# zongh5a/MDF-Net

Measured on AMD Instinct MI355X. Metric: views/sec at DTU 1600x1200x5-view x4-scale, higher is better.
Workload: dtype f32; 1 GPU; DTU eval 1600x1184 (1600x1200 cropped as load/dtueval.py:34), 5 views, 3 cost-volume stages + x2 refine = 4 output scales, hypotheses (48,24,8), batch 1 per rank, seeded random weights (pth/dtu_29.pth is not available offline); parallelism=views sharded over 1 rank(s), no collective

## Files before the change

include/mdfnet_hip.h:

```cpp
#ifndef MDFNET_HIP_H
#define MDFNET_HIP_H

#include <stdint.h>

#ifdef __cplusplus
extern "C" {
#endif

#define MDF_ABI_VERSION 1

#define MDF_OK 0
#define MDF_EARG (-1)
#define MDF_EUNSUPPORTED (-2)
#define MDF_EHIP (-3)

#define MDF_FEA_NCHW 0
#define MDF_FEA_NHWC 1
#define MDF_VOL_NCDHW 0
#define MDF_VOL_NDHWC 1

#define MDF_MAX_SRC_VIEWS 16
#define MDF_MAX_FUSE_VIEWS 1024

int mdf_abi_version(void);
const char* mdf_last_error(void);
const char* mdf_last_launch(void);
int mdf_release_stream(void* stream);

int mdf_homo_warp_fwd(const float* src_fea, int fea_layout, const float* proj, const float* hypos,
                      int hypos_per_pixel, float* out, int out_layout, int B, int C, int D, int h, int w,
                      void* stream);

int mdf_warp_corner_indices(const float* proj, const float* hypos, int hypos_per_pixel, int32_t* x0y0,
                            int B, int D, int h, int w, void* stream);

int mdf_warp_aggregate_vec_fwd(const float* ref_fea, const float* const* src_feas, int fea_layout,
                               const float* proj, const float* hypos, int hypos_per_pixel,
                               const float* w_params, float* cost, int cost_layout, int B, int C, int G,
                               int D, int h, int w, int n_src, void* stream);

int mdf_warp_aggregate_pairdiff_fwd(const float* ref_diff, const float* const* src_diffs, int fea_layout,
                                    const float* proj, const float* hypos, int hypos_per_pixel,
                                    const float* w_params, float* cost, int cost_layout, int B, int G, int D,
                                    int h, int w, int n_src, void* stream);

int mdf_warp_aggregate_var_fwd(const float* ref_fea, const float* const* src_feas, int fea_layout,
                               const float* proj, const float* hypos, int hypos_per_pixel, float* cost,
                               int cost_layout, int B, int C, int D, int h, int w, int n_src, void* stream);

int mdf_conv3d_fwd(const float* x, const float* wpack, const float* alpha, const float* beta, const float* res,
                   float* y, int B, int Di, int Hi, int Wi, int Cin, int Cout, int stride, int transposed,
                   int relu, void* stream);

int64_t mdf_conv3d_packed_size(int Cin, int Cout);
int mdf_conv3d_pack_weights(const float* w, float* wpack, int Cin, int Cout, int transposed, void* stream);

int mdf_conv2d_fwd(const float* x, const float* wpack, const float* alpha, const float* beta, const float* res,
                   float res_scale, const float* res_up, float* y, int B, int H, int W, int Cin, int Cout, int ksize, int stride, int relu,
                   int planar_in, int pixel_shuffle2, void* stream);
int64_t mdf_conv_packed_size(int Cin, int Cout, int ntaps);
int mdf_conv_pack_weights(const float* w, float* wpack, int Cin, int Cout, int ntaps, void* stream);

int mdf_prob_softmax_regress_fwd(const float* x, const float* w, const float* hypos, int hypos_per_pixel,
                                 float* prob, float* depth, int B, int D, int h, int wd, int Cin, void* stream);
int mdf_prob_from_partials_fwd(const float* partials, const float* hypos, int hypos_per_pixel, float* prob, float* depth,
                               int B, int D, int h, int wd, void* stream);
int mdf_prob_fused_fwd(const float* x, const float* wpack, const float* hypos, int hypos_per_pixel, float* prob, float* depth,
                       int B, int D, int h, int wd, int Cin, void* stream);

int mdf_refine_tail_fwd(const float* x, const float* w1pack, const float* w2, const float* lo, const float* span, float* y,
                        int B, int H, int W, void* stream);

int mdf_conv2d_pair_fwd(const float* x, const float* w1pack, const float* alpha1, const float* beta1, const float* w2pack,
                        const float* alpha2, const float* beta2, float* y, int N, int H, int W, void* stream);

int mdf_conv1x1_heads_fwd(const float* x, int n_heads, const float* const* wpacks, const float* const* biases,
                          const float* const* res_ups, float* const* ys, const int* couts, int B, int H, int W, int Cin,
                          void* stream);

int mdf_refine_head_fwd(const float* depth, const float* lo, const float* span, const float* weight, float* y, int B, int H, int W,
                        void* stream);

int mdf_conv2d_res_pair_fwd(const float* x, const float* wa_pack, const float* wb_pack, float scale, float* y, int N, int H,
                            int W, void* stream);

int mdf_depth_regress_fwd(const float* prob, const float* hypos, int hypos_per_pixel, float* depth, int B, int D,
                          int h, int w, void* stream);

int mdf_confidence_fwd(const float* prob, float* conf, int64_t* idx_out, int B, int D, int h, int w, void* stream);
int mdf_confidence_up2_fwd(const float* prob, float* conf2, int B, int D, int h, int w, void* stream);
int mdf_range_affine_fwd(const float* x, const float* lo, const float* span, int mode, float* y, int B, long long n, void* stream);

int mdf_hypos_fit_fwd(int mode, const float* prob, const float* depth, const float* hypos, int hypos_per_pixel,
                      const float* fit_row, float* s_out, int B, int D, int h, int w, void* stream);
int mdf_hypos_from_fit_fwd(int mode, const float* s, const float* depth, const float* range, float log_thresh,
                           float* hypos_out, int B, int D_out, int h, int w, int upsample, void* stream);

int mdf_consistency_fuse_fwd(const float* depth_ref, const float* conf, const float* const* src_depths, const float* mats,
                             int n_src, int h, int w, float photo_threshold, int nconditions, float thre1, float thre2,
                             float* depth_avg, unsigned char* masks, unsigned short* view_masks, float* rep_out, void* stream);

long long mdf_consensus_fuse_workspace(int n, int h, int w);
int mdf_consensus_fuse_fwd(const float* depths, const unsigned char* colors, const float* cams, int n, int h, int w, float f,
                           float disp_thresh, int num_consistent, void* workspace, float* xyz, unsigned char* rgb,
                           long long capacity, int* view_counts, long long* total, void* stream);
int mdf_consensus_compact(void* workspace, int n, int h, int w, float* xyz, unsigned char* rgb, long long capacity, void* stream);

#define MDF_PCD_MAX_SOURCES 64
#define MDF_PCD_STEP_VIS1 1
#define MDF_PCD_STEP_FUSION 2
#define MDF_PCD_STEP_VIS2 3
#define MDF_PCD_STEP_AVE 4
#define MDF_PCD_STEP_VIS3 5
#define MDF_PCD_STEP_SEG 6
long long mdf_pcd_fuse_workspace(int n, int h, int w, int v);
int mdf_pcd_fuse_fwd(float* depths, unsigned char* masks, const float* cams, const int* srcs, int n, int h, int w, int v, int need,
                     int first_step, int last_step, void* workspace, int* view_counts, long long* total, void* stream);
int mdf_pcd_compact(const float* depths, const unsigned char* masks, const unsigned char* rgb, const float* cams, int n, int h,
                    int w, int v, void* workspace, float* xyz, unsigned char* rgb_out, float* dirs, long long capacity,
                    void* stream);

long long mdf_pts_index_workspace(long long n);
int mdf_pts_index_build(const double* pts, long long n, void* index, long long index_bytes, void* stream);
int mdf_pts_nn_dist(const void* index, long long n, long long index_bytes, const void* qindex, const double* queries, long long m,
                    long long qindex_bytes, const double* bb, double cap, double* dist, int* visits, void* stream);
long long mdf_pts_reduce_workspace(long long n);
int mdf_pts_reduce_count(const void* index, long long n, long long index_bytes, const int* rank, double dst, void* workspace,
                         long long ws_bytes, long long* edges, void* stream);
int mdf_pts_reduce(const void* index, long long n, long long index_bytes, const int* rank, double dst, void* workspace,
                   long long ws_bytes, int* csr, long long capacity, int resume, int max_rounds, unsigned char* keep, int* state,
                   void* stream);
int mdf_dtu_masks(const double* qdata, long long n, const unsigned char* obs_mask, int s1, int s2, int s3, const double* bb,
                  double res, unsigned char* in_mask, const double* qstl, long long m, const double* plane, unsigned char* above,
                  void* stream);


int mdf_bn_stats_fwd(const float* y, long long N, int C, int ngroups, double* sums, void* stream);
int mdf_bn_finalize_fwd(const double* sums, const float* gamma, const float* beta, float eps, float momentum, long long N,
                        int C, int ngroups, float* aux, float* running_mean, float* running_var,
                        long long* num_batches_tracked, int nslices, void* stream);
int mdf_bn_relu_apply_fwd(const float* y, const float* aux, const float* res, float* z, long long N, int C, int ngroups,
                          void* stream);
int mdf_bn_finalize_apply_fwd(const float* y, const double* sums, const float* gamma, const float* beta, float eps, float momentum,
                              const float* res, float* z, float* aux, float* running_mean, float* running_var,
                              long long* num_batches_tracked, long long N, int C, int ngroups, int nslices, void* stream);
int mdf_bn_relu_bwd_reduce(const float* dz, const float* y, const float* aux, long long N, int C, int ngroups, double* red,
                           void* stream);
int mdf_bn_relu_bwd(const float* dz, const float* y, const float* aux, const double* red, const float* gamma, long long N,
                    int C, int ngroups, float* dy, float* dgamma, float* dbeta, int nslices, void* stream);

int64_t mdf_conv3d_wgrad_workspace(int B, int Ds, int Hs, int Ws, int A, int Bc);
// ... 85 lines not shown
```

mdf-net_amd/csrc/prob_fused.hip:

```cpp
#include "conv_lds_common.h"

namespace {

struct ProbParams {
  const float* x;
  const float* wpack;
  const float* hypos;
  int per_pixel;
  float* prob;
  float* depth;
  int B, D, H, W, tiles_h, tiles_w;
};

template <int CIN, int NW>
struct ProbCfg : Cfg<CIN, CIN, 4, 1, 3, 1, 1, 4> {
  typedef Cfg<CIN, CIN, 4, 1, 3, 1, 1, 4> Base;
  static constexpr int TH = NW, PH = NW + 2;
  static constexpr int S = round_s(PH * Base::PW, Base::KPL, Base::SW);
  static constexpr int PLANE = CIN * S;
  static constexpr int NTHR = 64 * NW;
  static constexpr int NFILL = (Base::NG * PH * Base::PW + NTHR - 1) / NTHR;
};

template <int CIN, int NW, int DT>
__global__ __launch_bounds__(64 * NW) void prob_fused_kernel(const ProbParams p) {
  typedef ProbCfg<CIN, NW> C;
  constexpr int KPL = C::KPL, NG = C::NG, S = C::S, PW = C::PW, PH = C::PH, NTHR = C::NTHR;
  typedef typename VecT<KPL>::type vec_t;
  extern __shared__ __attribute__((aligned(16))) float lds[];
  const int tid = threadIdx.x, lane = tid & 63, wave = tid >> 6;
  const int q = lane >> 4, n16 = lane & 15;
  const __amdgpu_buffer_rsrc_t wres = make_rsrc(p.wpack, (unsigned)(C::NSTEP * C::NT * 64 * KPL * 4));
  const int wvoff = lane * KPL * 4;
  const int lane_lds = (q * S + wave * PW + n16 * C::SW) * KPL;
  float wfirst[2][C::NT][KPL], wr[C::WN][C::NT][KPL];
#pragma unroll
  for (int i = 0; i < 2; ++i) {
    if constexpr (!C::WREG) buf_load_to<KPL>(wres, wvoff, i * (64 * KPL * 4), wfirst[i][0]);
    else {
#pragma unroll
      for (int k = 0; k < KPL; ++k) wfirst[i][0][k] = 0.f;
    }
  }
  if constexpr (C::WREG) {
#pragma unroll
    for (int i = 0; i < C::NSTEP; ++i) buf_load_to<KPL>(wres, wvoff, i * (64 * KPL * 4), wr[i][0]);
  } else {
#pragma unroll
    for (int k = 0; k < KPL; ++k) wr[0][0][k] = 0.f;
  }
  int sp = blockIdx.x;
  const int twi = sp % p.tiles_w; sp /= p.tiles_w;
  const int th = sp % p.tiles_h;
  const int b = sp / p.tiles_h;
  const int th0 = th * C::TH, tw0 = twi * C::TWO;

  constexpr int GF2 = (NG < 4) ? NG : 4;
  auto split2 = [&](int idx, int& v, int& g) {
    const int glo = idx % GF2, r = idx / GF2;
    v = r % (PH * PW);
    g = (r / (PH * PW)) * GF2 + glo;
  };
  auto load2 = [&](int idx, int d) -> vec_t {
    int g, v;
    split2(idx, v, g);
    const int row = v / PW, col = v - row * PW;
    const int ih = th0 - 1 + row, iw = tw0 - 1 + col;
    if (idx >= NG * PH * PW || ih < 0 || ih >= p.H || iw < 0 || iw >= p.W) return vec_zero<KPL>();
    return *reinterpret_cast<const vec_t*>(p.x + ((((size_t)b * p.D + d) * p.H + ih) * p.W + iw) * CIN + g * KPL);
  };
  auto store2 = [&](int idx, int slot, const vec_t& val) {
    if (idx < NG * PH * PW) {
      int g, v;
      split2(idx, v, g);
      *reinterpret_cast<vec_t*>(lds + slot * C::PLANE + (g * S + v) * KPL) = val;
    }
  };
#pragma unroll
  for (int k = 0; k < C::NFILL; ++k) store2(tid + k * NTHR, 0, load2(tid + k * NTHR, 0));
  __syncthreads();

  const int oh = th0 + wave, ow = tw0 + 4 * n16 + q;
  const bool row_live = oh < p.H;
  const bool live = row_live && ow < p.W;
  const size_t hw = (size_t)p.H * p.W;
  const size_t pix = live ? (size_t)oh * p.W + ow : 0;
  float* pr = p.prob + (size_t)b * p.D * hw + pix;
  float* lg = lds + 2 * C::PLANE + tid;
  float hy[DT ? DT : 1];
  if constexpr (DT != 0) {
    if (p.depth && live) {
#pragma unroll
      for (int d = 0; d < DT; ++d) hy[d] = p.per_pixel ? p.hypos[((size_t)b * DT + d) * hw + pix] : p.hypos[(size_t)b * DT + d];
    }
  }
  float carry1 = 0.f, carry0 = 0.f;
  float mx = -INFINITY;
  for (int d = 0; d < p.D; ++d) {
    const int slot = d & 1;
    const bool more = d + 1 < p.D;
    vec_t pf[C::NFILL];
    if (more) {
#pragma unroll
      for (int k = 0; k < C::NFILL; ++k) pf[k] = load2(tid + k * NTHR, d + 1);
    }
    if (row_live) {
      const float* planes[1] = {lds + slot * C::PLANE + lane_lds};
      f32x4 acc[1][C::NT];
      step_mfma<C, 1, 3, 1>(planes, wres, wvoff, wr, wfirst, acc);
      const float done = carry1 + acc[0][0][2];
      if (d >= 1) { lg[(d - 1) * NTHR] = done; mx = fmaxf(mx, done); }
      carry1 = carry0 + acc[0][0][1];
      carry0 = acc[0][0][0];
    }
    if (more) {
#pragma unroll
      for (int k = 0; k < C::NFILL; ++k) store2(tid + k * NTHR, slot ^ 1, pf[k]);
      __syncthreads();
    }
  }
  if (!live) return;
  lg[(p.D - 1) * NTHR] = carry1;
  mx = fmaxf(mx, carry1);
  float sum = 0.f;
  for (int d = 0; d < p.D; ++d) {
    const float e = expf(lg[d * NTHR] - mx);
    lg[d * NTHR] = e;
    sum += e;
  }
  mdf::CascadeSum dep;
  if constexpr (DT != 0) {
#pragma unroll
    for (int d = 0; d < DT; ++d) {
      const float pv = lg[d * NTHR] / sum;
      pr[(size_t)d * hw] = pv;
      if (p.depth) dep.add(pv * hy[d]);
    }
  } else {
    for (int d = 0; d < p.D; ++d) {
      const float pv = lg[d * NTHR] / sum;
      pr[(size_t)d * hw] = pv;
      if (p.depth) dep.add(pv * (p.per_pixel ? p.hypos[((size_t)b * p.D + d) * hw + pix] : p.hypos[(size_t)b * p.D + d]));
    }
  }
  if (p.depth) p.depth[(size_t)b * hw + pix] = dep.result();
}

template <int CIN, int NW, int DT>
int launch_prob_fused_d(ProbParams& p, hipStream_t st) {
  typedef ProbCfg<CIN, NW> C;
  const size_t kLds = ((size_t)2 * C::PLANE + (size_t)p.D * C::NTHR) * sizeof(float);
  if (kLds > 160 * 1024) return mdf::fail(MDF_EUNSUPPORTED, "fused prob head: D=%d does not fit the LDS (use the two-launch route)", p.D);
  p.tiles_h = (p.H + C::TH - 1) / C::TH;
  p.tiles_w = (p.W + C::TWO - 1) / C::TWO;
  const long long tiles = (long long)p.B * p.tiles_h * p.tiles_w;
  if (tiles > 0x7fffffff) return mdf::fail(MDF_EARG, "prob head: too many tiles");
  static bool attr_done_dev[64] = {};
  int dev_id = 0;
  (void)hipGetDevice(&dev_id);
  bool& attr_done = attr_done_dev[(dev_id >= 0 && dev_id < 64) ? dev_id : 0];
  if (!attr_done || dev_id >= 64) {
    hipError_t e = hipFuncSetAttribute(reinterpret_cast<const void*>(&prob_fused_kernel<CIN, NW, DT>), hipFuncAttributeMaxDynamicSharedMemorySize, 160 * 1024);
    if (e != hipSuccess) return mdf::fail(MDF_EHIP, "hipFuncSetAttribute(dynamic LDS): %s", hipGetErrorString(e));
    attr_done = true;
  }
  hipLaunchKernelGGL((prob_fused_kernel<CIN, NW, DT>), dim3((unsigned)tiles), dim3(C::NTHR), kLds, st, p);
  return mdf::check_launch("prob_fused_kernel");
}

template <int CIN, int NW>
int launch_prob_fused(ProbParams& p, hipStream_t st) {
  if (p.D == 24) return launch_prob_fused_d<CIN, NW, 24>(p, st);
  if (p.D == 8) return launch_prob_fused_d<CIN, NW, 8>(p, st);
  return launch_prob_fused_d<CIN, NW, 0>(p, st);
}

}

extern "C" int mdf_prob_fused_fwd(const float* x, const float* wpack, const float* hypos, int hypos_per_pixel, float* prob, float* depth,
                                  int B, int D, int h, int wd, int Cin, void* stream) {
  MDF_REQUIRE(x && wpack && prob, "null pointer argument");
  MDF_REQUIRE(depth == nullptr || hypos != nullptr, "depth output needs hypos");
  MDF_REQUIRE(B > 0 && D > 0 && h > 0 && wd > 0, "bad shape");
  MDF_REQUIRE((long long)B * D * h * wd * Cin < (1ll << 31), "input too large for 32-bit offsets");
  ProbParams p{};
  p.x = x; p.hypos = hypos; p.per_pixel = hypos_per_pixel; p.prob = prob; p.depth = depth; p.B = B; p.D = D; p.H = h; p.W = wd;
  p.wpack = wpack + (size_t)9 * Cin * 16;
  if (Cin == 8) return launch_prob_fused<8, 4>(p, (hipStream_t)stream);
  if (Cin == 16) return launch_prob_fused<16, 4>(p, (hipStream_t)stream);
  return mdf::fail(MDF_EUNSUPPORTED, "fused prob head is built for Cin in {8,16}, got %d", Cin);
}
```

mdf-net_amd/mdfnet_hip/__init__.py:

```python
import ctypes
import os
import threading

import torch

_PKG = os.path.dirname(os.path.abspath(__file__))
LIB_PATH = os.environ.get("MDF_HIP_LIB") or os.path.join(_PKG, "libmdfnet_hip.so")
ABI_VERSION = 1

_lib = None
_lock = threading.Lock()

c_fp = ctypes.c_void_p
c_int = ctypes.c_int
c_i64 = ctypes.c_int64

SIGNATURES = {
    "mdf_abi_version": (c_int, []),
    "mdf_last_error": (ctypes.c_char_p, []),
    "mdf_last_launch": (ctypes.c_char_p, []),
    "mdf_release_stream": (c_int, [c_fp]),
    "mdf_homo_warp_fwd": (c_int, [c_fp, c_int, c_fp, c_fp, c_int, c_fp, c_int] + [c_int] * 5 + [c_fp]),
    "mdf_warp_corner_indices": (c_int, [c_fp, c_fp, c_int, c_fp] + [c_int] * 4 + [c_fp]),
    "mdf_warp_aggregate_vec_fwd": (c_int, [c_fp, ctypes.POINTER(c_fp), c_int, c_fp, c_fp, c_int, c_fp, c_fp, c_int]
                                   + [c_int] * 7 + [c_fp]),
    "mdf_warp_aggregate_pairdiff_fwd": (c_int, [c_fp, ctypes.POINTER(c_fp), c_int, c_fp, c_fp, c_int, c_fp, c_fp, c_int]
                                        + [c_int] * 6 + [c_fp]),
    "mdf_warp_aggregate_var_fwd": (c_int, [c_fp, ctypes.POINTER(c_fp), c_int, c_fp, c_fp, c_int, c_fp, c_int]
                                   + [c_int] * 6 + [c_fp]),
    "mdf_conv3d_fwd": (c_int, [c_fp] * 6 + [c_int] * 9 + [c_fp]),
    "mdf_conv3d_packed_size": (c_i64, [c_int, c_int]),
    "mdf_conv3d_pack_weights": (c_int, [c_fp, c_fp, c_int, c_int, c_int, c_fp]),
    "mdf_conv2d_fwd": (c_int, [c_fp] * 5 + [ctypes.c_float, c_fp, c_fp] + [c_int] * 10 + [c_fp]),
    "mdf_conv2d_pair_fwd": (c_int, [c_fp] * 8 + [c_int] * 3 + [c_fp]),
    "mdf_conv1x1_heads_fwd": (c_int, [c_fp, c_int, ctypes.POINTER(c_fp), ctypes.POINTER(c_fp), ctypes.POINTER(c_fp), ctypes.POINTER(c_fp),
                                      ctypes.POINTER(c_int)] + [c_int] * 4 + [c_fp]),
    "mdf_refine_head_fwd": (c_int, [c_fp] * 5 + [c_int] * 3 + [c_fp]),
    "mdf_conv2d_res_pair_fwd": (c_int, [c_fp] * 3 + [ctypes.c_float, c_fp] + [c_int] * 3 + [c_fp]),
    "mdf_refine_tail_fwd": (c_int, [c_fp] * 6 + [c_int] * 3 + [c_fp]),
    "mdf_conv_packed_size": (c_i64, [c_int, c_int, c_int]),
    "mdf_conv_pack_weights": (c_int, [c_fp, c_fp, c_int, c_int, c_int, c_fp]),
    "mdf_prob_softmax_regress_fwd": (c_int, [c_fp, c_fp, c_fp, c_int, c_fp, c_fp] + [c_int] * 5 + [c_fp]),
    "mdf_prob_from_partials_fwd": (c_int, [c_fp, c_fp, c_int, c_fp, c_fp] + [c_int] * 4 + [c_fp]),
    "mdf_prob_fused_fwd": (c_int, [c_fp, c_fp, c_fp, c_int, c_fp, c_fp] + [c_int] * 5 + [c_fp]),
    "mdf_depth_regress_fwd": (c_int, [c_fp, c_fp, c_int, c_fp] + [c_int] * 4 + [c_fp]),
    "mdf_confidence_fwd": (c_int, [c_fp, c_fp, c_fp] + [c_int] * 4 + [c_fp]),
    "mdf_confidence_up2_fwd": (c_int, [c_fp, c_fp] + [c_int] * 4 + [c_fp]),
    "mdf_range_affine_fwd": (c_int, [c_fp, c_fp, c_fp, c_int, c_fp, c_int, c_i64, c_fp]),
    "mdf_hypos_fit_fwd": (c_int, [c_int, c_fp, c_fp, c_fp, c_int, c_fp, c_fp] + [c_int] * 4 + [c_fp]),
    "mdf_consistency_fuse_fwd": (c_int, [c_fp, c_fp, ctypes.POINTER(c_fp), c_fp, c_int, c_int, c_int, ctypes.c_float, c_int,
                                         ctypes.c_float, ctypes.c_float, c_fp, c_fp, c_fp, c_fp, c_fp]),
    "mdf_consensus_fuse_workspace": (c_i64, [c_int, c_int, c_int]),
    "mdf_consensus_fuse_fwd": (c_int, [c_fp, c_fp, c_fp, c_int, c_int, c_int, ctypes.c_float, ctypes.c_float, c_int, c_fp, c_fp, c_fp,
                                       c_i64, c_fp, c_fp, c_fp]),
    "mdf_consensus_compact": (c_int, [c_fp, c_int, c_int, c_int, c_fp, c_fp, c_i64, c_fp]),
    "mdf_pcd_fuse_workspace": (c_i64, [c_int, c_int, c_int, c_int]),
    "mdf_pcd_fuse_fwd": (c_int, [c_fp, c_fp, c_fp, c_fp] + [c_int] * 7 + [c_fp, c_fp, c_fp, c_fp]),
    "mdf_pcd_compact": (c_int, [c_fp, c_fp, c_fp, c_fp] + [c_int] * 4 + [c_fp, c_fp, c_fp, c_fp, c_i64, c_fp]),
    "mdf_pts_index_workspace": (c_i64, [c_i64]),
    "mdf_pts_index_build": (c_int, [c_fp, c_i64, c_fp, c_i64, c_fp]),
    "mdf_pts_nn_dist": (c_int, [c_fp, c_i64, c_i64, c_fp, c_fp, c_i64, c_i64, ctypes.POINTER(ctypes.c_double), ctypes.c_double, c_fp,
                                c_fp, c_fp]),
    "mdf_pts_reduce_workspace": (c_i64, [c_i64]),
    "mdf_pts_reduce_count": (c_int, [c_fp, c_i64, c_i64, c_fp, ctypes.c_double, c_fp, c_i64, c_fp, c_fp]),
    "mdf_pts_reduce": (c_int, [c_fp, c_i64, c_i64, c_fp, ctypes.c_double, c_fp, c_i64, c_fp, c_i64, c_int, c_int, c_fp, c_fp, c_fp]),
    "mdf_dtu_masks": (c_int, [c_fp, c_i64, c_fp, c_int, c_int, c_int, ctypes.POINTER(ctypes.c_double), ctypes.c_double, c_fp, c_fp,
                              c_i64, ctypes.POINTER(ctypes.c_double), c_fp, c_fp]),
    "mdf_bn_stats_fwd": (c_int, [c_fp, c_i64, c_int, c_int, c_fp, c_fp]),
    "mdf_bn_finalize_fwd": (c_int, [c_fp, c_fp, c_fp, ctypes.c_float, ctypes.c_float, c_i64, c_int, c_int, c_fp, c_fp, c_fp, c_fp, c_int, c_fp]),
    "mdf_bn_relu_apply_fwd": (c_int, [c_fp, c_fp, c_fp, c_fp, c_i64, c_int, c_int, c_fp]),
    "mdf_bn_finalize_apply_fwd": (c_int, [c_fp, c_fp, c_fp, c_fp, ctypes.c_float, ctypes.c_float, c_fp, c_fp, c_fp, c_fp, c_fp, c_fp, c_i64, c_int, c_int, c_int, c_fp]),
    "mdf_bn_relu_bwd_reduce": (c_int, [c_fp, c_fp, c_fp, c_i64, c_int, c_int, c_fp, c_fp]),
    "mdf_bn_relu_bwd": (c_int, [c_fp, c_fp, c_fp, c_fp, c_fp, c_i64, c_int, c_int, c_fp, c_fp, c_fp, c_int, c_fp]),
    "mdf_conv3d_wgrad_workspace": (c_i64, [c_int] * 6),
    "mdf_conv3d_wgrad": (c_int, [c_fp] * 4 + [c_int] * 8 + [c_fp]),
    "mdf_conv3d_train_fwd": (c_int, [c_fp] * 4 + [c_int] * 9 + [c_fp] * 3 + [c_int, c_fp]),
    "mdf_conv2d_train_fwd": (c_int, [c_fp] * 3 + [c_int] * 9 + [c_fp] * 3 + [c_int, c_int, c_fp]),
    "mdf_conv3d_wgrad_partial": (c_int, [c_fp] * 4 + [c_int] * 7 + [ctypes.POINTER(c_int), c_fp]),
    "mdf_conv2d_wgrad_partial": (c_int, [c_fp] * 4 + [c_int] * 7 + [ctypes.POINTER(c_int), c_fp]),
    "mdf_wgrad_sum_batch": (c_int, [ctypes.POINTER(c_fp), ctypes.POINTER(c_fp), ctypes.POINTER(c_int), ctypes.POINTER(c_int), c_int, c_fp]),
    "mdf_wgrad_batch_begin": (c_int, []),
    "mdf_wgrad_batch_flush": (c_int, [c_fp]),
    "mdf_conv2d_wgrad_workspace": (c_i64, [c_int] * 6),
    "mdf_conv2d_wgrad": (c_int, [c_fp] * 4 + [c_int] * 8 + [c_fp]),
    "mdf_pack_job_bytes": (c_i64, []),
    "mdf_pack_job_fill": (c_i64, [c_fp, c_int, c_fp, c_fp] + [c_int] * 9),
    "mdf_pack_batch": (c_int, [c_fp, c_fp, c_int, c_fp]),
    "mdf_upsample2_bilinear_bwd": (c_int, [c_fp, c_fp] + [c_int] * 5 + [c_fp]),
    "mdf_prob_softmax_regress_bwd": (c_int, [c_fp, c_fp, c_int, c_fp, c_fp, c_fp] + [c_int] * 4 + [c_fp]),
    "mdf_prob_conv_dgrad": (c_int, [c_fp, c_fp, c_fp] + [c_int] * 5 + [c_fp]),
    "mdf_prob_conv_dgrad_stat": (c_int, [c_fp, c_fp, c_fp] + [c_int] * 5 + [c_fp, c_fp, c_fp, c_int, c_fp]),
    "mdf_warp_aggregate_vec_train": (c_int, [c_int, c_fp, ctypes.POINTER(c_fp), c_fp, c_fp, c_int, c_fp, c_fp, c_fp, c_fp, c_fp, c_fp,
                                             c_fp, ctypes.POINTER(c_fp), c_fp, c_fp] + [c_int] * 7 + [c_fp]),
    "mdf_aggregate_train_prepare": (c_int, [c_fp] * 4 + [c_i64, c_int, c_int, c_fp, c_fp, c_int, c_fp]),
    "mdf_aggregate_train_finalize": (c_int, [c_fp] * 3 + [ctypes.c_float, ctypes.c_float, c_i64, c_int, c_int] + [c_fp] * 5),
    "mdf_aggregate_train_bwd_finalize": (c_int, [c_fp, c_fp, c_int, c_i64, c_fp, c_fp, c_fp, c_fp, c_i64, c_fp]),
    "mdf_warp_aggregate_var_bwd": (c_int, [c_fp, ctypes.POINTER(c_fp), c_fp, c_fp, c_int, c_fp, c_fp, ctypes.POINTER(c_fp)]
                                   + [c_int] * 6 + [c_fp]),
    "mdf_homo_warp_bwd": (c_int, [c_fp, c_int, c_fp, c_fp, c_int, c_fp] + [c_int] * 5 + [c_fp]),
    "mdf_masked_smooth_l1_reduce": (c_int, [c_fp, c_fp, c_fp, c_int, c_int, c_int, c_i64, c_fp, c_fp]),
    "mdf_masked_smooth_l1_finalize": (c_int, [c_fp, c_int, c_fp, c_fp, c_fp]),
    "mdf_masked_smooth_l1_bwd": (c_int, [c_fp, c_fp, c_fp, c_int, c_int, c_int, c_i64, c_fp, c_fp, c_fp, c_fp]),
    "mdf_masked_smooth_l1_reduce_multi": (c_int, [ctypes.POINTER(c_fp), ctypes.POINTER(c_fp), ctypes.POINTER(c_i64), c_int, c_fp, c_int, c_int, c_int, c_fp, c_fp]),
    "mdf_masked_smooth_l1_bwd_multi": (c_int, [ctypes.POINTER(c_fp), ctypes.POINTER(c_fp), ctypes.POINTER(c_i64), c_int, c_fp, c_int, c_int, c_int, c_fp, c_fp,
                                               ctypes.POINTER(c_fp), c_fp]),
    "mdf_fpn_compose_fwd": (c_int, [c_fp] * 6 + [c_int] * 3 + [c_fp, c_fp]),
    "mdf_fpn_compose_bwd": (c_int, [c_fp] * 14 + [c_int] * 3 + [c_fp] * 7),
    "mdf_adam_job_bytes": (c_i64, []),
    "mdf_adam_job_fill": (c_i64, [c_fp, c_int, c_fp, c_i64, c_i64, c_int]),
    "mdf_adam_step": (c_int, [c_fp, c_fp, c_int, c_fp, c_fp, c_fp] + [ctypes.c_float] * 5 + [c_i64, c_fp]),
    "mdf_adam_step_hyper": (c_int, [c_fp, c_fp, c_int, c_fp, c_fp, c_fp, c_fp] + [ctypes.c_float] * 4 + [c_fp]),
    "mdf_hypos_from_fit_fwd": (c_int, [c_int, c_fp, c_fp, c_fp, ctypes.c_float, c_fp] + [c_int] * 5 + [c_fp]),
}


class MdfHipError(RuntimeError):
    pass


def lib():
    global _lib
    if _lib is None:
        with _lock:
            if _lib is None:
                if not os.path.exists(LIB_PATH):
                    raise MdfHipError(
                        f"{LIB_PATH} not found: the HIP extension is not built and there is no fallback path. "
# ... 27 lines not shown
```

mdf-net_amd/mdfnet_hip/ops.py:

```python
import ctypes
import os
import threading

import torch

from . import check, lib

FEA_NHWC = 1
VOL_NCDHW, VOL_NDHWC = 0, 1

_prof = None


def profile_begin():
    global _prof
    _prof = []


def profile_end():
    global _prof
    recs, _prof = _prof, None
    torch.cuda.synchronize()
    return [(n, tag, e0.elapsed_time(e1), work) for n, tag, e0, e1, work in recs]

# ... 315 lines not shown

def conv3d_ndhwc(x, wpack, cin, cout, stride=1, transposed=False, alpha=None, beta=None, relu=False, res=None):
    _need_gpu(x, wpack)
    b, d, h, w, c = x.shape
    assert c == cin and x.is_contiguous()
    if transposed:
        do, ho, wo = 2 * d, 2 * h, 2 * w
    elif stride == 2:
        do, ho, wo = (d - 1) // 2 + 1, (h - 1) // 2 + 1, (w - 1) // 2 + 1
    else:
        do, ho, wo = d, h, w
    y = torch.empty((b, do, ho, wo, cout), device=x.device, dtype=torch.float32)
    if res is not None:
        assert res.shape == y.shape and res.is_contiguous()
    _abi("mdf_conv3d_fwd", (x.data_ptr(), wpack.data_ptr(), None if alpha is None else alpha.data_ptr(),
                               None if beta is None else beta.data_ptr(), None if res is None else res.data_ptr(),
                               y.data_ptr(), b, d, h, w, cin, cout, stride, int(transposed), int(relu), _stream(y),),
         tag=f"{cin}->{cout} {'T' if transposed else 's%d' % stride} {d}x{h}x{w}",
         work={"flops": 2.0 * 27 * cin * cout * b * (d * h * w if transposed else do * ho * wo),
               "bytes": 4.0 * (x.numel() + y.numel() * (2 if res is not None else 1)), "bound": "mfma"})
    return y


STAT_SLICES = 16


def conv3d_train(x, wpack, cin, cout, stride, transposed, res, stat_mode, stat_out, stat_y=None, stat_aux=None):
    _need_gpu(x, wpack, stat_out)
    b, d, h, w, c = x.shape
    assert c == cin and x.is_contiguous()
    if transposed:
        do, ho, wo = 2 * d, 2 * h, 2 * w
    elif stride == 2:
        do, ho, wo = (d - 1) // 2 + 1, (h - 1) // 2 + 1, (w - 1) // 2 + 1
    else:
        do, ho, wo = d, h, w
    y = torch.empty((b, do, ho, wo, cout), device=x.device, dtype=torch.float32)
    if res is not None:
        assert res.shape == y.shape and res.is_contiguous()
    if stat_mode == 2:
        assert stat_y.shape == y.shape and stat_y.is_contiguous() and stat_aux.numel() == 4 * cout
    nslices = stat_out.numel() // (2 * cout)
    assert stat_out.numel() == nslices * 2 * cout and stat_out.dtype == torch.float64
    _abi("mdf_conv3d_train_fwd", (x.data_ptr(), wpack.data_ptr(), None if res is None else res.data_ptr(), y.data_ptr(), b, d, h, w, cin, cout,
                                  stride, int(transposed), stat_mode, None if stat_y is None else stat_y.data_ptr(),
                                  None if stat_aux is None else stat_aux.data_ptr(), stat_out.data_ptr(), nslices, _stream(y)),
         tag=f"{cin}->{cout} {'T' if transposed else 's%d' % stride} {d}x{h}x{w} +sums{stat_mode}",
         work={"flops": 2.0 * 27 * cin * cout * b * (d * h * w if transposed else do * ho * wo),
               "bytes": 4.0 * (x.numel() + y.numel() * (1 + (res is not None) + (stat_mode == 2))), "bound": "mfma"})
    return y


def conv2d_train(x, wpack, cin, cout, ksize, stride, planar_in, stat_mode, stat_out, ngroups, stat_y=None, stat_aux=None):
    _need_gpu(x, wpack, stat_out)
    if planar_in:
        b, c, h, w = x.shape
    else:
        b, h, w, c = x.shape
    assert c == cin and x.is_contiguous() and b % ngroups == 0
    pad = (ksize - 1) // 2
    ho, wo = (h + 2 * pad - ksize) // stride + 1, (w + 2 * pad - ksize) // stride + 1
    y = torch.empty((b, ho, wo, cout), device=x.device, dtype=torch.float32)
    if stat_mode == 2:
        assert stat_y.shape == y.shape and stat_y.is_contiguous() and stat_aux.numel() == ngroups * 4 * cout
    nslices = stat_out.numel() // (ngroups * 2 * cout)
    assert stat_out.numel() == nslices * ngroups * 2 * cout and stat_out.dtype == torch.float64
    _abi("mdf_conv2d_train_fwd", (x.data_ptr(), wpack.data_ptr(), y.data_ptr(), b, h, w, cin, cout, ksize, stride, int(planar_in), stat_mode,
                                  None if stat_y is None else stat_y.data_ptr(), None if stat_aux is None else stat_aux.data_ptr(),
                                  stat_out.data_ptr(), nslices, ngroups, _stream(y)),
         tag=f"{cin}->{cout} k{ksize}s{stride} {h}x{w}x{b} +sums{stat_mode}",
         work={"flops": 2.0 * ksize * ksize * cin * cout * b * ho * wo, "bytes": 4.0 * (x.numel() + y.numel() * (1 + (stat_mode == 2))),
               "bound": "mfma"})
    return y


def pack_prob_weight(weight):
    w = weight.detach().float()
    w2 = torch.zeros((4, w.shape[1], 3, 3), device=w.device, dtype=torch.float32)
    w2[:3] = w[0].permute(1, 0, 2, 3)
    return pack_conv2d_weight(w2)


PROB_FUSED = os.environ.get("MDF_PROB_FUSED", "1") != "0"
PROB_FUSED_MIN_TILES = int(os.environ.get("MDF_PROB_FUSED_MIN_TILES", "400"))


def prob_head(x, weight, depth_hypos=None, direct=False, wpack=None):
    _need_gpu(x, weight)
    b, d, h, w, c = x.shape
    prob = torch.empty((b, d, h, w), device=x.device, dtype=torch.float32)
    depth, hyp, pp = None, None, 0
    if depth_hypos is not None:
        hyp, pp = _hypos_arg(depth_hypos, h, w)
        depth = torch.empty((b, h, w), device=x.device, dtype=torch.float32)
    fused_lds = 2 * c * 398 * 4 + d * 1024
    if (not direct and c in (8, 16) and x.is_contiguous() and PROB_FUSED and fused_lds <= 160 * 1024
            and b * ((h + 3) // 4) * ((w + 63) // 64) >= PROB_FUSED_MIN_TILES):
        wp = pack_prob_weight(weight) if wpack is None else wpack
        _abi("mdf_prob_fused_fwd", (x.data_ptr(), wp.data_ptr(), None if hyp is None else hyp.data_ptr(), pp, prob.data_ptr(),
                                    None if depth is None else depth.data_ptr(), b, d, h, w, c, _stream(prob),),
             tag=f"{c}->1 {d}x{h}x{w}", work={"flops": 2.0 * 27 * c * b * d * h * w,
                                              "bytes": 4.0 * (x.numel() + prob.numel()), "bound": "hbm"})
        return prob if depth is None else (prob, depth)
    if not direct and c in (8, 16) and d <= 96 and x.is_contiguous():
        part = conv2d_nhwc(x.view(b * d, h, w, c), pack_prob_weight(weight) if wpack is None else wpack, c, 4, 3, 1,
                           useful_cout=3)
        _abi("mdf_prob_from_partials_fwd", (part.data_ptr(), None if hyp is None else hyp.data_ptr(), pp, prob.data_ptr(),
                                            None if depth is None else depth.data_ptr(), b, d, h, w, _stream(prob),),
             tag=f"partials->prob {d}x{h}x{w}", work={"bytes": 4.0 * (part.numel() + prob.numel()), "bound": "hbm"})
        return prob if depth is None else (prob, depth)
    _abi("mdf_prob_softmax_regress_fwd", (x.data_ptr(), _f32c(weight.detach()).data_ptr(),
                                             None if hyp is None else hyp.data_ptr(), pp, prob.data_ptr(),
                                             None if depth is None else depth.data_ptr(), b, d, h, w, c, _stream(prob),),
         tag=f"{c}->1 {d}x{h}x{w}", work={"flops": 2.0 * 27 * c * b * d * h * w,
                                          "bytes": 4.0 * (x.numel() + prob.numel()), "bound": "hbm"})
    return prob if depth is None else (prob, depth)


def refine_tail(x, w1pack, w2, lo=None, span=None):
    _need_gpu(x, w1pack, w2)
    b, h, w, c = x.shape
    assert c == 8 and x.is_contiguous() and tuple(w2.shape) == (1, 8, 3, 3)
    y = torch.empty((b, 2 * h, 2 * w), device=x.device, dtype=torch.float32)
    w2_c, lo_c, span_c = _f32c(w2.detach()), (None if lo is None else _f32c(lo)), (None if span is None else _f32c(span))
    _abi("mdf_refine_tail_fwd", (x.data_ptr(), w1pack.data_ptr(), w2_c.data_ptr(), None if lo_c is None else lo_c.data_ptr(),
                                 None if span_c is None else span_c.data_ptr(), y.data_ptr(), b, h, w, _stream(y),),
         tag=f"8->32->1 {h}x{w}x{b}", work={"flops": 2.0 * 72 * (32 + 4) * b * h * w, "bytes": 4.0 * (x.numel() + y.numel()), "bound": "mfma"})
    return y


def fold_bn(bn_weight, bn_bias, running_mean, running_var, eps=1e-5):
    invstd = 1.0 / torch.sqrt(running_var.float() + eps)
    alpha = (bn_weight.float() * invstd).contiguous()
    beta = (bn_bias.float() - running_mean.float() * alpha).contiguous()
    return alpha, beta


def pack_conv2d_weight(w):
    _need_gpu(w)
    cout, cin, k, _ = w.shape
    n = lib().mdf_conv_packed_size(cin, cout, k * k)
    out = torch.empty((n,), device=w.device, dtype=torch.float32)
    _abi("mdf_conv_pack_weights", (_f32c(w.detach()).data_ptr(), out.data_ptr(), cin, cout, k * k, _stream(out),))
    return out


def conv2d_nhwc(x, wpack, cin, cout, ksize, stride=1, alpha=None, beta=None, relu=False, res=None, res_scale=1.0,
                res_up=None, planar_in=False, useful_cout=None, pixel_shuffle2=False):
    _need_gpu(x, wpack)
    if planar_in:
        b, c, h, w = x.shape
    else:
        b, h, w, c = x.shape
    assert c == cin and x.is_contiguous()
    pad = (ksize - 1) // 2
    ho, wo = (h + 2 * pad - ksize) // stride + 1, (w + 2 * pad - ksize) // stride + 1
    y = torch.empty((b, 2 * ho, 2 * wo, cout // 4) if pixel_shuffle2 else (b, ho, wo, cout), device=x.device, dtype=torch.float32)
    _abi("mdf_conv2d_fwd", (x.data_ptr(), wpack.data_ptr(), None if alpha is None else alpha.data_ptr(),
                            None if beta is None else beta.data_ptr(), None if res is None else res.data_ptr(),
                            ctypes.c_float(res_scale), None if res_up is None else res_up.data_ptr(), y.data_ptr(),
                            b, h, w, cin, cout, ksize, stride, int(relu), int(planar_in), int(pixel_shuffle2), _stream(y),),
         tag=f"{cin}->{cout} k{ksize}s{stride} {h}x{w}x{b}",
         work={"flops": 2.0 * ksize * ksize * cin * (useful_cout or cout) * b * ho * wo, "bytes": 4.0 * (x.numel() + y.numel()),
               "bound": "mfma"})
    return y


def conv2d_pair_planar(x, w1pack, a1, b1, w2pack, a2, b2):
    _need_gpu(x, w1pack, w2pack)
    n, c, h, w = x.shape
    assert c == 3 and x.is_contiguous() and x.dtype == torch.float32
    y = torch.empty((n, h, w, 8), device=x.device, dtype=torch.float32)
    _abi("mdf_conv2d_pair_fwd", (x.data_ptr(), w1pack.data_ptr(), a1.data_ptr(), b1.data_ptr(), w2pack.data_ptr(), a2.data_ptr(), b2.data_ptr(),
                                 y.data_ptr(), n, h, w, _stream(y)), tag=f"3->8->8 k3 {h}x{w}x{n}",
         work={"flops": 2.0 * 9 * (3 * 8 + 8 * 8) * n * h * w, "bytes": 4.0 * (x.numel() + y.numel()), "bound": "mfma"})
    return y


def conv1x1_heads(x, heads, res_ups):
    _need_gpu(x)
# ... 403 lines not shown
```

Before: 299.8 views/s.

## Split fused prob head depth loop across wave segments with LDS weights

The fused probability-head kernel now splits the depth dimension across several wave segments in one block. Each segment streams its own depth range and stitches the 3-tap depth convolution at segment boundaries through LDS. The softmax max, sum and depth regression are reduced across segments, and for Cin=16 the weights are staged in LDS rather than re-read from global memory. It also adds XCD block remapping, an optional register prefetch queue, a query for the LDS size, and lowers the minimum tile count for taking the fused path. This should expose more parallelism for small tile counts, at the cost of extra barriers and more LDS per block.

Result: no change. 299.4 views/s (-0.1%).

```diff
diff --git a/include/mdfnet_hip.h b/include/mdfnet_hip.h
--- a/include/mdfnet_hip.h
+++ b/include/mdfnet_hip.h
@@ -67,6 +67,7 @@
                                int B, int D, int h, int wd, void* stream);
 int mdf_prob_fused_fwd(const float* x, const float* wpack, const float* hypos, int hypos_per_pixel, float* prob, float* depth,
                        int B, int D, int h, int wd, int Cin, void* stream);
+long long mdf_prob_fused_lds_bytes(int B, int D, int h, int wd, int Cin);
 
 int mdf_refine_tail_fwd(const float* x, const float* w1pack, const float* w2, const float* lo, const float* span, float* y,
                         int B, int H, int W, void* stream);
diff --git a/mdf-net_amd/csrc/prob_fused.hip b/mdf-net_amd/csrc/prob_fused.hip
--- a/mdf-net_amd/csrc/prob_fused.hip
+++ b/mdf-net_amd/csrc/prob_fused.hip
@@ -10,38 +10,67 @@
   float* prob;
   float* depth;
   int B, D, H, W, tiles_h, tiles_w;
+  int remap;
 };
 
-template <int CIN, int NW>
+constexpr int HMAX = 24;
+
+template <int CIN, int NW, int NSEG, int RING>
 struct ProbCfg : Cfg<CIN, CIN, 4, 1, 3, 1, 1, 4> {
   typedef Cfg<CIN, CIN, 4, 1, 3, 1, 1, 4> Base;
+  static_assert(RING == 1 || RING == 2, "one slot + registers, or two slots");
   static constexpr int TH = NW, PH = NW + 2;
   static constexpr int S = round_s(PH * Base::PW, Base::KPL, Base::SW);
   static constexpr int PLANE = CIN * S;
-  static constexpr int NTHR = 64 * NW;
-  static constexpr int NFILL = (Base::NG * PH * Base::PW + NTHR - 1) / NTHR;
+  static constexpr int NPIX = 64 * NW;
+  static constexpr int NTHR = NPIX * NSEG;
+  static constexpr int NFILL = (Base::NG * PH * Base::PW + NPIX - 1) / NPIX;
+  static constexpr int LG_OFF = NSEG * RING * PLANE;
+  static constexpr int WL = Base::WREG ? 0 : Base::NSTEP * 64 * Base::KPL;
+  static size_t lds_bytes(int D) { return ((size_t)LG_OFF + (size_t)D * NPIX + (size_t)3 * NSEG * NPIX + WL) * sizeof(float); }
 };
 
-template <int CIN, int NW, int DT>
-__global__ __launch_bounds__(64 * NW) void prob_fused_kernel(const ProbParams p) {
-  typedef ProbCfg<CIN, NW> C;
-  constexpr int KPL = C::KPL, NG = C::NG, S = C::S, PW = C::PW, PH = C::PH, NTHR = C::NTHR;
+template <typename C>
+__device__ __forceinline__ void step_mfma_wlds(const float* plane, const float* wl, f32x4& acc) {
+  constexpr int KPL = C::KPL, NCH = C::NCH, S = C::S, PW = C::PW, NSTEP = C::NSTEP;
+  static_assert(C::NT == 1, "one n-tile");
+  acc = (f32x4){0.f, 0.f, 0.f, 0.f};
+  float af[2][KPL], bf[2][KPL];
+  auto load = [&](int i, int buf) {
+    const int ch = i % NCH, tap = i / NCH;
+    const int kw = tap % C::KW, kh = tap / C::KW;
+    lds_frag<KPL>(wl + i * (64 * KPL), af[buf]);
+    lds_frag<KPL>(plane + ((ch * 4) * S + kh * PW + kw) * KPL, bf[buf]);
+  };
+  load(0, 0);
+#pragma unroll
+  for (int i = 0; i < NSTEP; ++i) {
+    if (i + 1 < NSTEP) load(i + 1, (i + 1) & 1);
+    __builtin_amdgcn_sched_barrier(0);
+#pragma unroll
+    for (int s = 0; s < KPL; ++s) acc = __builtin_amdgcn_mfma_f32_16x16x4f32(af[i & 1][s], bf[i & 1][s], acc, 0, 0, 0);
+    __builtin_amdgcn_sched_barrier(0);
+  }
+}
+
+template <int CIN, int NW, int NSEG, int RING, int PD>
+__global__ __launch_bounds__(64 * NW * NSEG) void prob_fused_kernel(const ProbParams p) {
+  typedef ProbCfg<CIN, NW, NSEG, RING> C;
+  constexpr int KPL = C::KPL, NG = C::NG, S = C::S, PW = C::PW, PH = C::PH, NPIX = C::NPIX;
   typedef typename VecT<KPL>::type vec_t;
   extern __shared__ __attribute__((aligned(16))) float lds[];
   const int tid = threadIdx.x, lane = tid & 63, wave = tid >> 6;
+  const int seg = wave / NW, row = wave - seg * NW;
+  const int stid = tid - seg * NPIX;
   const int q = lane >> 4, n16 = lane & 15;
   const __amdgpu_buffer_rsrc_t wres = make_rsrc(p.wpack, (unsigned)(C::NSTEP * C::NT * 64 * KPL * 4));
   const int wvoff = lane * KPL * 4;
-  const int lane_lds = (q * S + wave * PW + n16 * C::SW) * KPL;
+  const int lane_lds = (q * S + row * PW + n16 * C::SW) * KPL;
   float wfirst[2][C::NT][KPL], wr[C::WN][C::NT][KPL];
 #pragma unroll
-  for (int i = 0; i < 2; ++i) {
-    if constexpr (!C::WREG) buf_load_to<KPL>(wres, wvoff, i * (64 * KPL * 4), wfirst[i][0]);
-    else {
-#pragma unroll
-      for (int k = 0; k < KPL; ++k) wfirst[i][0][k] = 0.f;
-    }
-  }
+  for (int i = 0; i < 2; ++i)
+#pragma unroll
+    for (int k = 0; k < KPL; ++k) wfirst[i][0][k] = 0.f;
   if constexpr (C::WREG) {
 #pragma unroll
     for (int i = 0; i < C::NSTEP; ++i) buf_load_to<KPL>(wres, wvoff, i * (64 * KPL * 4), wr[i][0]);
@@ -49,11 +78,15 @@
 #pragma unroll
     for (int k = 0; k < KPL; ++k) wr[0][0][k] = 0.f;
   }
-  int sp = blockIdx.x;
+  int sp = p.remap ? (int)mdf::xcd_remap(blockIdx.x, gridDim.x) : (int)blockIdx.x;
   const int twi = sp % p.tiles_w; sp /= p.tiles_w;
   const int th = sp % p.tiles_h;
   const int b = sp / p.tiles_h;
   const int th0 = th * C::TH, tw0 = twi * C::TWO;
+
+  const int L = (p.D + NSEG - 1) / NSEG;
+  const int d0 = min(seg * L, p.D), d1 = min(d0 + L, p.D), len = d1 - d0;
+  float* ring = lds + seg * (RING * C::PLANE);
 
   constexpr int GF2 = (NG < 4) ? NG : 4;
   auto split2 = [&](int idx, int& v, int& g) {
@@ -64,8 +97,8 @@
   auto load2 = [&](int idx, int d) -> vec_t {
     int g, v;
     split2(idx, v, g);
-    const int row = v / PW, col = v - row * PW;
-    const int ih = th0 - 1 + row, iw = tw0 - 1 + col;
+    const int prow = v / PW, col = v - prow * PW;
+    const int ih = th0 - 1 + prow, iw = tw0 - 1 + col;
     if (idx >= NG * PH * PW || ih < 0 || ih >= p.H || iw < 0 || iw >= p.W) return vec_zero<KPL>();
     return *reinterpret_cast<const vec_t*>(p.x + ((((size_t)b * p.D + d) * p.H + ih) * p.W + iw) * CIN + g * KPL);
   };
@@ -73,84 +106,183 @@
     if (idx < NG * PH * PW) {
       int g, v;
       split2(idx, v, g);
-      *reinterpret_cast<vec_t*>(lds + slot * C::PLANE + (g * S + v) * KPL) = val;
+      *reinterpret_cast<vec_t*>(ring + slot * C::PLANE + (g * S + v) * KPL) = val;
     }
   };
-#pragma unroll
-  for (int k = 0; k < C::NFILL; ++k) store2(tid + k * NTHR, 0, load2(tid + k * NTHR, 0));
-  __syncthreads();
-
-  const int oh = th0 + wave, ow = tw0 + 4 * n16 + q;
+  vec_t queue[PD > 0 ? PD : 1][C::NFILL];
+  {
+    vec_t first[C::NFILL];
+#pragma unroll
+    for (int k = 0; k < C::NFILL; ++k) first[k] = (len > 0) ? load2(stid + k * NPIX, d0) : vec_zero<KPL>();
+#pragma unroll
+    for (int j = 0; j < PD; ++j)
+#pragma unroll
+      for (int k = 0; k < C::NFILL; ++k) queue[j][k] = (d0 + 1 + j < d1) ? load2(stid + k * NPIX, d0 + 1 + j) : vec_zero<KPL>();
+    if (len > 0) {
+#pragma unroll
+      for (int k = 0; k < C::NFILL; ++k) store2(stid + k * NPIX, 0, first[k]);
+    }
+  }
+
+  const int oh = th0 + row, ow = tw0 + 4 * n16 + q;
   const bool row_live = oh < p.H;
   const bool live = row_live && ow < p.W;
   const size_t hw = (size_t)p.H * p.W;
   const size_t pix = live ? (size_t)oh * p.W + ow : 0;
   float* pr = p.prob + (size_t)b * p.D * hw + pix;
-  float* lg = lds + 2 * C::PLANE + tid;
-  float hy[DT ? DT : 1];
-  if constexpr (DT != 0) {
-    if (p.depth && live) {
-#pragma unroll
-      for (int d = 0; d < DT; ++d) hy[d] = p.per_pixel ? p.hypos[((size_t)b * DT + d) * hw + pix] : p.hypos[(size_t)b * DT + d];
-    }
-  }
+  float* lg = lds + C::LG_OFF + stid;
+  float* xp0 = lg + (size_t)p.D * NPIX;
+  float* xp2 = xp0 + NSEG * NPIX;
+  float* smx = xp2 + NSEG * NPIX;
+  const float* wl = smx + NSEG * NPIX - stid + lane * KPL;
+  if constexpr (!C::WREG) {
+    float* wdst = smx + NSEG * NPIX - stid;
+    for (int i = tid; i < C::WL / KPL; i += C::NTHR) {
+      float v[KPL];
+      buf_load_to<KPL>(wres, i * KPL * 4, 0, v);
+#pragma unroll
+      for (int k = 0; k < KPL; ++k) wdst[i * KPL + k] = v[k];
+    }
+  }
+  auto hypo_at = [&](int d) -> float { return p.per_pixel ? p.hypos[((size_t)b * p.D + d) * hw + pix] : p.hypos[(size_t)b * p.D + d]; };
+  const bool hy_reg = L <= HMAX;
+  float hy[HMAX] = {};
+  if (p.depth && live && hy_reg) {
+#pragma unroll
+    for (int i = 0; i < HMAX; ++i)
+      if (i < len) hy[i] = hypo_at(d0 + i);
+  }
+  __syncthreads();
+
   float carry1 = 0.f, carry0 = 0.f;
+  float first_p1 = 0.f, first_p2n = 0.f;
   float mx = -INFINITY;
-  for (int d = 0; d < p.D; ++d) {
-    const int slot = d & 1;
-    const bool more = d + 1 < p.D;
+  for (int it = 0; it < L; ++it) {
+    const int d = d0 + it;
+    const int slot = (RING == 2) ? (it & 1) : 0;
+    const bool more = d + 1 < d1, fetch = d + 1 + PD < d1;
     vec_t pf[C::NFILL];
-    if (more) {
-#pragma unroll
-      for (int k = 0; k < C::NFILL; ++k) pf[k] = load2(tid + k * NTHR, d + 1);
-    }
-    if (row_live) {
-      const float* planes[1] = {lds + slot * C::PLANE + lane_lds};
+#pragma unroll
+    for (int k = 0; k < C::NFILL; ++k) pf[k] = fetch ? load2(stid + k * NPIX, d + 1 + PD) : vec_zero<KPL>();
+    if (row_live && d < d1) {
+      const float* planes[1] = {ring + slot * C::PLANE + lane_lds};
       f32x4 acc[1][C::NT];
-      step_mfma<C, 1, 3, 1>(planes, wres, wvoff, wr, wfirst, acc);
-      const float done = carry1 + acc[0][0][2];
-      if (d >= 1) { lg[(d - 1) * NTHR] = done; mx = fmaxf(mx, done); }
-      carry1 = carry0 + acc[0][0][1];
+      if constexpr (C::WREG) step_mfma<C, 1, 3, 1>(planes, wres, wvoff, wr, wfirst, acc);
+      else step_mfma_wlds<C>(planes[0], wl, acc[0][0]);
+      if (it == 0) {
+        first_p1 = acc[0][0][1];
+        xp2[seg * NPIX] = acc[0][0][2];
+      } else if (it == 1) {
+        first_p2n = acc[0][0][2];
+        carry1 = carry0 + acc[0][0][1];
+      } else {
+        const float done = carry1 + acc[0][0][2];
+        lg[(d - 1) * NPIX] = done;
+        mx = fmaxf(mx, done);
+        carry1 = carry0 + acc[0][0][1];
+      }
       carry0 = acc[0][0][0];
     }
-    if (more) {
-#pragma unroll
-      for (int k = 0; k < C::NFILL; ++k) store2(tid + k * NTHR, slot ^ 1, pf[k]);
+    if (it + 1 < L) {
+      if constexpr (RING == 1) __syncthreads();
+      if (more) {
+#pragma unroll
+        for (int k = 0; k < C::NFILL; ++k) store2(stid + k * NPIX, (RING == 2) ? (slot ^ 1) : 0, PD > 0 ? queue[0][k] : pf[k]);
+      }
       __syncthreads();
     }
-  }
-  if (!live) return;
-  lg[(p.D - 1) * NTHR] = carry1;
-  mx = fmaxf(mx, carry1);
+    if constexpr (PD > 0) {
+#pragma unroll
+      for (int k = 0; k < C::NFILL; ++k) {
+#pragma unroll
+        for (int j = 0; j + 1 < PD; ++j) queue[j][k] = queue[j + 1][k];
+        queue[PD - 1][k] = pf[k];
+      }
+    }
+  }
+  if (row_live && len > 0) xp0[seg * NPIX] = carry0;
+  __syncthreads();
+
+  if (row_live && len > 0) {
+    const float a = (d0 > 0 ? xp0[(seg - 1) * NPIX] : 0.f) + first_p1;
+    if (len >= 2) {
+      const float l0 = a + first_p2n;
+      const float l1 = (d1 < p.D) ? carry1 + xp2[(seg + 1) * NPIX] : carry1;
+      lg[d0 * NPIX] = l0;
+      lg[(d1 - 1) * NPIX] = l1;
+      mx = fmaxf(mx, fmaxf(l0, l1));
+    } else {
+      const float l0 = (d1 < p.D) ? a + xp2[(seg + 1) * NPIX] : a;
+      lg[d0 * NPIX] = l0;
+      mx = fmaxf(mx, l0);
+    }
+  }
+  smx[seg * NPIX] = mx;
+  __syncthreads();
+  mx = smx[0];
+#pragma unroll
+  for (int s = 1; s < NSEG; ++s) mx = fmaxf(mx, smx[s * NPIX]);
+  for (int d = d0; d < d1; ++d) lg[d * NPIX] = expf(lg[d * NPIX] - mx);
+  __syncthreads();
   float sum = 0.f;
-  for (int d = 0; d < p.D; ++d) {
-    const float e = expf(lg[d * NTHR] - mx);
-    lg[d * NTHR] = e;
-    sum += e;
-  }
-  mdf::CascadeSum dep;
-  if constexpr (DT != 0) {
-#pragma unroll
-    for (int d = 0; d < DT; ++d) {
-      const float pv = lg[d * NTHR] / sum;
-      pr[(size_t)d * hw] = pv;
-      if (p.depth) dep.add(pv * hy[d]);
-    }
-  } else {
-    for (int d = 0; d < p.D; ++d) {
-      const float pv = lg[d * NTHR] / sum;
-      pr[(size_t)d * hw] = pv;
-      if (p.depth) dep.add(pv * (p.per_pixel ? p.hypos[((size_t)b * p.D + d) * hw + pix] : p.hypos[(size_t)b * p.D + d]));
-    }
-  }
-  if (p.depth) p.depth[(size_t)b * hw + pix] = dep.result();
-}
-
-template <int CIN, int NW, int DT>
-int launch_prob_fused_d(ProbParams& p, hipStream_t st) {
-  typedef ProbCfg<CIN, NW> C;
-  const size_t kLds = ((size_t)2 * C::PLANE + (size_t)p.D * C::NTHR) * sizeof(float);
-  if (kLds > 160 * 1024) return mdf::fail(MDF_EUNSUPPORTED, "fused prob head: D=%d does not fit the LDS (use the two-launch route)", p.D);
+  for (int d = 0; d < p.D; ++d) sum += lg[d * NPIX];
+  if (!p.depth) {
+    if (live)
+      for (int d = d0; d < d1; ++d) pr[(size_t)d * hw] = lg[d * NPIX] / sum;
+    return;
+  }
+  __syncthreads();
+  if (live) {
+    if (hy_reg) {
+#pragma unroll
+      for (int i = 0; i < HMAX; ++i)
+        if (i < len) {
+          const float pv = lg[(d0 + i) * NPIX] / sum;
+          pr[(size_t)(d0 + i) * hw] = pv;
+          lg[(d0 + i) * NPIX] = pv * hy[i];
+        }
+    } else {
+      for (int d = d0; d < d1; ++d) {
+        const float pv = lg[d * NPIX] / sum;
+        pr[(size_t)d * hw] = pv;
+        lg[d * NPIX] = pv * hypo_at(d);
+      }
+    }
+  }
+  __syncthreads();
+  if (seg == 0 && live) {
+    mdf::CascadeSum dep;
+    for (int d = 0; d < p.D; ++d) dep.add(lg[d * NPIX]);
+    p.depth[(size_t)b * hw + pix] = dep.result();
+  }
+}
+
+struct ProbForm { int nw, nseg, ring, pd; };
+constexpr size_t kLdsMax = 160 * 1024;
+
+size_t form_lds_bytes(const ProbForm& f, int Cin, int D) {
+  const int kpl = Cin >= 16 ? 4 : 2, s = round_s((f.nw + 2) * 66, kpl, 4), npix = 64 * f.nw;
+  const int wl = Cin >= 16 ? 18 * 64 * kpl : 0;
+  return ((size_t)f.nseg * f.ring * Cin * s + (size_t)D * npix + (size_t)3 * f.nseg * npix + wl) * sizeof(float);
+}
+
+int pick_forms(int Cin, int B, int D, int h, int wd, ProbForm (&out)[4]) {
+  int n = 0;
+  if (const char* e = getenv("MDF_PROB_FORM")) {
+    ProbForm f{0, 0, 0, 0};
+    if (sscanf(e, "%d,%d,%d,%d", &f.nw, &f.nseg, &f.ring, &f.pd) == 4) out[n++] = f;
+  }
+  (void)B; (void)h; (void)wd;
+  if (Cin == 16) out[n++] = ProbForm{3, 4, 1, 0};
+  out[n++] = ProbForm{4, 1, 2, 0};
+  return n;
+}
+
+template <int CIN, int NW, int NSEG, int RING, int PD>
+int launch_prob_form(ProbParams& p, hipStream_t st) {
+  typedef ProbCfg<CIN, NW, NSEG, RING> C;
+  const size_t kLds = C::lds_bytes(p.D);
+  if (kLds > kLdsMax) return mdf::fail(MDF_EUNSUPPORTED, "fused prob head: D=%d does not fit the LDS (use the two-launch route)", p.D);
   p.tiles_h = (p.H + C::TH - 1) / C::TH;
   p.tiles_w = (p.W + C::TWO - 1) / C::TWO;
   const long long tiles = (long long)p.B * p.tiles_h * p.tiles_w;
@@ -160,21 +292,44 @@
   (void)hipGetDevice(&dev_id);
   bool& attr_done = attr_done_dev[(dev_id >= 0 && dev_id < 64) ? dev_id : 0];
   if (!attr_done || dev_id >= 64) {
-    hipError_t e = hipFuncSetAttribute(reinterpret_cast<const void*>(&prob_fused_kernel<CIN, NW, DT>), hipFuncAttributeMaxDynamicSharedMemorySize, 160 * 1024);
+    hipError_t e = hipFuncSetAttribute(reinterpret_cast<const void*>(&prob_fused_kernel<CIN, NW, NSEG, RING, PD>), hipFuncAttributeMaxDynamicSharedMemorySize, (int)kLdsMax);
     if (e != hipSuccess) return mdf::fail(MDF_EHIP, "hipFuncSetAttribute(dynamic LDS): %s", hipGetErrorString(e));
     attr_done = true;
   }
-  hipLaunchKernelGGL((prob_fused_kernel<CIN, NW, DT>), dim3((unsigned)tiles), dim3(C::NTHR), kLds, st, p);
+  { const char* e = getenv("MDF_PROB_REMAP"); p.remap = e ? atoi(e) : 1; }
+  hipLaunchKernelGGL((prob_fused_kernel<CIN, NW, NSEG, RING, PD>), dim3((unsigned)tiles), dim3(C::NTHR), kLds, st, p);
   return mdf::check_launch("prob_fused_kernel");
 }
 
-template <int CIN, int NW>
+#define MDF_PROB_FORMS(X) X(4, 1, 2, 0) X(4, 1, 2, 1) X(3, 4, 1, 0)
+
+template <int CIN>
 int launch_prob_fused(ProbParams& p, hipStream_t st) {
-  if (p.D == 24) return launch_prob_fused_d<CIN, NW, 24>(p, st);
-  if (p.D == 8) return launch_prob_fused_d<CIN, NW, 8>(p, st);
-  return launch_prob_fused_d<CIN, NW, 0>(p, st);
-}
-
+  ProbForm forms[4];
+  const int n = pick_forms(CIN, p.B, p.D, p.H, p.W, forms);
+  for (int i = 0; i < n; ++i) {
+    const ProbForm& f = forms[i];
+    if (form_lds_bytes(f, CIN, p.D) > kLdsMax) continue;
+#define MDF_PROB_CASE(NW, NSEG, RING, PD) \
+    if (f.nw == NW && f.nseg == NSEG && f.ring == RING && f.pd == PD) return launch_prob_form<CIN, NW, NSEG, RING, PD>(p, st);
+    MDF_PROB_FORMS(MDF_PROB_CASE)
+#undef MDF_PROB_CASE
+    return mdf::fail(MDF_EUNSUPPORTED, "fused prob head: form %d,%d,%d,%d is not built", f.nw, f.nseg, f.ring, f.pd);
+  }
+  return mdf::fail(MDF_EUNSUPPORTED, "fused prob head: D=%d does not fit the LDS (use the two-launch route)", p.D);
+}
+
+}
+
+extern "C" long long mdf_prob_fused_lds_bytes(int B, int D, int h, int wd, int Cin) {
+  if ((Cin != 8 && Cin != 16) || B <= 0 || D <= 0 || h <= 0 || wd <= 0) return 0;
+  ProbForm forms[4];
+  const int n = pick_forms(Cin, B, D, h, wd, forms);
+  for (int i = 0; i < n; ++i) {
+    const size_t need = form_lds_bytes(forms[i], Cin, D);
+    if (need <= kLdsMax) return (long long)need;
+  }
+  return 0;
 }
 
 extern "C" int mdf_prob_fused_fwd(const float* x, const float* wpack, const float* hypos, int hypos_per_pixel, float* prob, float* depth,
@@ -186,7 +341,7 @@
   ProbParams p{};
   p.x = x; p.hypos = hypos; p.per_pixel = hypos_per_pixel; p.prob = prob; p.depth = depth; p.B = B; p.D = D; p.H = h; p.W = wd;
   p.wpack = wpack + (size_t)9 * Cin * 16;
-  if (Cin == 8) return launch_prob_fused<8, 4>(p, (hipStream_t)stream);
-  if (Cin == 16) return launch_prob_fused<16, 4>(p, (hipStream_t)stream);
+  if (Cin == 8) return launch_prob_fused<8>(p, (hipStream_t)stream);
+  if (Cin == 16) return launch_prob_fused<16>(p, (hipStream_t)stream);
   return mdf::fail(MDF_EUNSUPPORTED, "fused prob head is built for Cin in {8,16}, got %d", Cin);
 }
diff --git a/mdf-net_amd/mdfnet_hip/__init__.py b/mdf-net_amd/mdfnet_hip/__init__.py
--- a/mdf-net_amd/mdfnet_hip/__init__.py
+++ b/mdf-net_amd/mdfnet_hip/__init__.py
@@ -43,6 +43,7 @@
     "mdf_prob_softmax_regress_fwd": (c_int, [c_fp, c_fp, c_fp, c_int, c_fp, c_fp] + [c_int] * 5 + [c_fp]),
     "mdf_prob_from_partials_fwd": (c_int, [c_fp, c_fp, c_int, c_fp, c_fp] + [c_int] * 4 + [c_fp]),
     "mdf_prob_fused_fwd": (c_int, [c_fp, c_fp, c_fp, c_int, c_fp, c_fp] + [c_int] * 5 + [c_fp]),
+    "mdf_prob_fused_lds_bytes": (c_i64, [c_int] * 5),
     "mdf_depth_regress_fwd": (c_int, [c_fp, c_fp, c_int, c_fp] + [c_int] * 4 + [c_fp]),
     "mdf_confidence_fwd": (c_int, [c_fp, c_fp, c_fp] + [c_int] * 4 + [c_fp]),
     "mdf_confidence_up2_fwd": (c_int, [c_fp, c_fp] + [c_int] * 4 + [c_fp]),
diff --git a/mdf-net_amd/mdfnet_hip/ops.py b/mdf-net_amd/mdfnet_hip/ops.py
--- a/mdf-net_amd/mdfnet_hip/ops.py
+++ b/mdf-net_amd/mdfnet_hip/ops.py
@@ -421,7 +421,7 @@
 
 
 PROB_FUSED = os.environ.get("MDF_PROB_FUSED", "1") != "0"
-PROB_FUSED_MIN_TILES = int(os.environ.get("MDF_PROB_FUSED_MIN_TILES", "400"))
+PROB_FUSED_MIN_TILES = int(os.environ.get("MDF_PROB_FUSED_MIN_TILES", "64"))
 
 
 def prob_head(x, weight, depth_hypos=None, direct=False, wpack=None):
@@ -432,9 +432,9 @@
     if depth_hypos is not None:
         hyp, pp = _hypos_arg(depth_hypos, h, w)
         depth = torch.empty((b, h, w), device=x.device, dtype=torch.float32)
-    fused_lds = 2 * c * 398 * 4 + d * 1024
-    if (not direct and c in (8, 16) and x.is_contiguous() and PROB_FUSED and fused_lds <= 160 * 1024
-            and b * ((h + 3) // 4) * ((w + 63) // 64) >= PROB_FUSED_MIN_TILES):
+    if (not direct and c in (8, 16) and x.is_contiguous() and PROB_FUSED
+            and b * ((h + 3) // 4) * ((w + 63) // 64) >= PROB_FUSED_MIN_TILES
+            and lib().mdf_prob_fused_lds_bytes(b, d, h, w, c) > 0):
         wp = pack_prob_weight(weight) if wpack is None else wpack
         _abi("mdf_prob_fused_fwd", (x.data_ptr(), wp.data_ptr(), None if hyp is None else hyp.data_ptr(), pp, prob.data_ptr(),
                                     None if depth is None else depth.data_ptr(), b, d, h, w, c, _stream(prob),),
```
